# jason2714/de-i2i-gan

Measured on AMD Instinct MI355X. Metric: paired 256x256 images/sec (G+D train step), higher is better.
Workload: dtype bf16

## Files before the change

### de-i2i-gan_amd/csrc/conv_api.hip

```cpp
#include <hip/hip_runtime.h>

#include "../../include/dei2i_hip.h"
#include "launch.h"

namespace dei2i {

static ConvShape to_shape(const dei2i_conv* c) {
  ConvShape s;
  s.N = c->N; s.H = c->H; s.W = c->W; s.Cin = c->Cin; s.Cout = c->Cout;
  s.kh = c->kh; s.kw = c->kw; s.stride = c->stride; s.pad = c->pad; s.pad_mode = c->pad_mode; s.up = c->up;
  return s;
}

static bool valid_conv(const dei2i_conv* c) {
  if (!c) return false;
  const int vec = c->dtype == DT_BF16 ? 8 : 4;
  if (c->dtype != DT_BF16 && c->dtype != DT_F32) return false;
  if (c->N <= 0 || c->H <= 0 || c->W <= 0 || c->Cin <= 0 || c->Cout <= 0) return false;
  if (c->CinS < c->Cin || c->CoutS < c->Cout || c->CinS % vec || c->CoutS % vec) return false;
  if (c->kh <= 0 || c->kw <= 0 || c->stride <= 0 || c->pad < 0 || c->up < 0 || c->up > 1) return false;
  if (c->kh < c->stride || c->kw < c->stride) return false;
  if (c->pad_mode == PAD_REFLECT && (c->pad >= (c->H << c->up) || c->pad >= (c->W << c->up))) return false;
  if (((c->H << c->up) + 2 * c->pad) < c->kh || ((c->W << c->up) + 2 * c->pad) < c->kw) return false;
  return true;
// ... 335 lines not shown
    hipError_t e = gather_gemm(c->dtype, interior, dy, wd_packed, c->Cin, nullptr, dx, ws, ws_bytes, c->CinS, ACT_NONE, st);
    if (e != hipSuccess) return (int)e;
    GatherDesc ring[4];
    reflect_ring_descs(ring_frame, c->H, c->W, p, c->kh, c->kw, ring);
    const long long woffs[4] = {0, 0, 0, 0};
    e = gather_gemm_multi(c->dtype, ring, woffs, 4, dy, wd_packed, c->Cin, nullptr, ext_scratch, ws, ws_bytes, c->CinS, ACT_NONE, st,
                          true);
    if (e != hipSuccess) return (int)e;
    return fold_border(c, ext_scratch, dx, p, st);
  }
  if (reflect && g_opt.dgrad_s2_ring && c->stride == 2 && c->kh == 4 && c->kw == 4 && p == 1 && !c->up && c->H % 2 == 0 && c->W % 2 == 0 &&
      c->H >= 8 && c->W >= 8 && (size_t)c->N * c->H * c->W * c->CinS >= ((size_t)48 << 20)) {
    ConvShape sh = to_shape(c);
    GatherDesc rows[4], cols[4], in4[4];
    long long wrows4[4], wcols4[4], woffs[4];
    s2_ring_descs(sh, c->CoutS, rows, wrows4, cols, wcols4);
    sh.pad_mode = PAD_ZERO;
    for_each_dgrad_class(c->Cin, c->CoutS, c->kh, c->kw, 2, [&](const DgradClass& k) {
      in4[2 * k.ay + k.ax] = make_dgrad_desc(sh, c->CoutS, k.ay, k.ax);
      woffs[2 * k.ay + k.ax] = k.off;
    });
    hipError_t e = gather_gemm_multi(c->dtype, in4, woffs, 4, dy, wd_packed, c->Cin, nullptr, dx, ws, ws_bytes, c->CinS, ACT_NONE, st);
    if (e != hipSuccess) return (int)e;
    e = gather_gemm_multi(c->dtype, rows, wrows4, 4, dy, wd_packed, c->Cin, nullptr, ext_scratch, ws, ws_bytes, c->CinS, ACT_NONE, st, true);
    if (e != hipSuccess) return (int)e;
    e = gather_gemm_multi(c->dtype, cols, wcols4, 4, dy, wd_packed, c->Cin, nullptr, ext_scratch, ws, ws_bytes, c->CinS, ACT_NONE, st, true);
    if (e != hipSuccess) return (int)e;
    return fold_border(c, ext_scratch, dx, 1, st);
  }
  const int rc = dei2i_conv2d_dgrad(c, dy, wd_packed, ext_scratch, ws, ws_bytes, s);
  if (rc != 0) return rc;
  return dei2i_fold_pad(c->dtype, c->N, c->H, c->W, c->CinS, c->pad, c->pad_mode, c->up, ext_scratch, nullptr, dx, s);
}

static GatherDesc interior_dgrad_desc(const dei2i_conv* c) {
  ConvShape sh = to_shape(c);
  sh.pad_mode = PAD_ZERO;
  return make_dgrad_desc(sh, c->CoutS, 0, 0);
}

static bool dgrad_norm_shape_ok(const dei2i_conv* c) {
  if (!g_opt.halo16 || !g_opt.halo16_fold) return false;
  if (!valid_conv(c) || c->dtype != DT_BF16 || c->up) return false;
  if (c->kh != 3 || c->kw != 3 || c->stride != 1 || c->pad != 1 || c->pad_mode != PAD_REFLECT) return false;
  return halo16_shape_ok(interior_dgrad_desc(c), c->CinS, true, true, false);
}

int dei2i_conv2d_dgrad_norm_supported(const dei2i_conv* c) { return dgrad_norm_shape_ok(c) ? 1 : 0; }

int dei2i_conv2d_dgrad_norm_chunks(const dei2i_conv* c) { return (c->H / 16) * (c->W / 32); }

int dei2i_conv2d_dgrad_input_norm(const dei2i_conv* c, const void* dy, const void* wd_packed, void* dx, const dei2i_epi_norm* en,
                                  dei2i_stream s) {
  if (!dy || !wd_packed || !dx || !en || !dgrad_norm_shape_ok(c)) return DEI2I_ERR_BAD_ARG;
  if (!en->x || !en->mean || !en->rstd || !en->partial || en->up < 0 || en->up > 1) return DEI2I_ERR_BAD_ARG;
  const int kind = en->kind;
  if (kind == 1 ? !en->gb : (kind != 2 || !en->a || !en->b || en->up)) return DEI2I_ERR_BAD_ARG;
  if (en->group_images < 0 || (en->group_images > 0 && c->N % en->group_images != 0)) return DEI2I_ERR_BAD_ARG;
  const GatherDesc interior = interior_dgrad_desc(c);
  EpiNorm e;
  e.x = (const uint16_t*)en->x; e.mean = en->mean; e.rstd = en->rstd; e.gb = (const uint16_t*)en->gb; e.a = en->a; e.b = en->b;
  e.partial = en->partial; e.kind = en->kind; e.up = en->up; e.act = en->act;
  e.group_images = kind == 2 ? en->group_images : 0;
  hipError_t ef = halo16_conv(interior, dy, wd_packed, c->Cin, nullptr, dx, c->CinS, ACT_NONE, (hipStream_t)s, nullptr, nullptr, true, &e);
  return ef == hipErrorNotSupported ? DEI2I_ERR_BAD_ARG : (int)ef;
}

int dei2i_conv2d_wgrad_oihw(const dei2i_conv* c, const void* x, const void* dy, float* scratch, size_t scratch_elems,
                            float* dw_oihw, int accumulate, dei2i_stream s) {
  if (!valid_conv(c) || !x || !dy || !scratch || !dw_oihw) return DEI2I_ERR_BAD_ARG;
  hipStream_t st = (hipStream_t)s;
  GatherDesc g = make_fwd_desc(to_shape(c), c->CinS);
  const size_t packed = (size_t)wgrad_slab_elems(c->Cout, g.K);
  if (scratch_elems < packed) return DEI2I_ERR_WORKSPACE;
  const bool bf16 = c->dtype == DT_BF16;
  int nsplit = 0;
  hipError_t e = hipErrorNotSupported;
  if (bf16 && g_opt.wgrad_thin)
    e = wgrad_thin(g, x, dy, c->Cout, c->CoutS, scratch, scratch_elems, &nsplit, st);
  if (e == hipErrorNotSupported && bf16 && g_opt.wgrad_halo)
    e = wgrad_halo(g, x, dy, c->Cout, c->CoutS, scratch, scratch_elems, &nsplit, g_opt.wgrad_halo == 2, st);
  if (e == hipErrorNotSupported && bf16 && g_opt.wgrad_v2)
    e = wgrad_v2(g, x, dy, c->Cout, c->CoutS, scratch, scratch_elems, &nsplit, st);
  if (e == hipErrorNotSupported) e = wgrad_gemm(c->dtype, g, x, dy, c->Cout, c->CoutS, scratch, scratch_elems, &nsplit, st);
  if (e != hipSuccess) return (int)e;
  return (int)wgrad_reduce_unpack(scratch, nsplit, (long long)packed, dw_oihw, c->Cout, c->Cin, c->CinS, c->kh * c->kw, accumulate, st);
}

static bool to_pro(const dei2i_conv* c, const dei2i_pro* p, ConvPro& out) {
  if (p == nullptr) return false;
  out.A = p->A; out.B = p->B; out.n_stride = p->n_stride; out.slope = p->slope;
  out.ring = (const uint16_t*)p->ring;
  out.ring_pix = p->ring != nullptr ? ring_pixels(c->H << c->up, c->W << c->up) : 0;
  return true;
}

static bool halo_fwd_shape_ok(const dei2i_conv* c, int want_pro) {
  if (!valid_conv(c) || c->dtype != DT_BF16) return false;
  if (c->kh == 4 && c->kw == 4 && c->stride == 2 && c->pad == 1 && !want_pro)
    return halo16_s2_shape_ok(make_fwd_desc(to_shape(c), c->CinS), c->CoutS);
  if (c->kh != 3 || c->kw != 3 || c->stride != 1 || c->pad != 1) return false;
  return halo_conv_shape_ok(make_fwd_desc(to_shape(c), c->CinS), c->CoutS, want_pro != 0, want_pro != 0);
}

int dei2i_conv2d_fused_supported(const dei2i_conv* c, int want_pro) { return halo_fwd_shape_ok(c, want_pro) ? 1 : 0; }

int dei2i_conv2d_stats_chunks(const dei2i_conv* c) {
  int Ho, Wo;
  dei2i_conv2d_out_shape(c, &Ho, &Wo);
  return (Ho / 8) * (Wo / 32);
}

int dei2i_conv2d_fwd_fused(const dei2i_conv* c, const void* x, const void* w_packed, const float* bias, int act, void* y,
                           const dei2i_pro* pro, float* stats, dei2i_stream s) {
  if (!x || !w_packed || !y || !halo_fwd_shape_ok(c, pro != nullptr)) return DEI2I_ERR_BAD_ARG;
  if (pro != nullptr && (!pro->A || !pro->B)) return DEI2I_ERR_BAD_ARG;
  GatherDesc g = make_fwd_desc(to_shape(c), c->CinS);
  ConvPro cp;
  const bool has = to_pro(c, pro, cp);
  if (!has) {
    hipError_t e = halo16_conv(g, x, w_packed, c->Cout, bias, y, c->CoutS, act, (hipStream_t)s, stats);
    if (e != hipErrorNotSupported) return (int)e;
  }
  return (int)halo_conv(g, x, w_packed, c->Cout, bias, y, c->CoutS, act, (hipStream_t)s, nullptr, has ? &cp : nullptr, stats);
}

int dei2i_conv2d_ring_supported(const dei2i_conv* c) {
  if (!halo_fwd_shape_ok(c, 0) || !c->up) return 0;
  return halo16_shape_ok(make_fwd_desc(to_shape(c), c->CinS), c->CoutS, false, false, true) ? 1 : 0;
}

int dei2i_conv2d_fwd_ring(const dei2i_conv* c, const void* z_src, const void* ring, const void* w_packed, const float* bias, int act,
                          void* y, float* stats, dei2i_stream s) {
  if (!z_src || !ring || !w_packed || !y || !dei2i_conv2d_ring_supported(c)) return DEI2I_ERR_BAD_ARG;
  GatherDesc g = make_fwd_desc(to_shape(c), c->CinS);
  return (int)halo16_conv(g, z_src, w_packed, c->Cout, bias, y, c->CoutS, act, (hipStream_t)s, stats, ring);
}

int dei2i_conv2d_wgrad_pro_supported(const dei2i_conv* c) {
  if (!valid_conv(c) || c->dtype != DT_BF16) return 0;
  if (c->kh != 3 || c->kw != 3 || c->stride != 1 || c->pad != 1) return 0;
  return wgrad_halo_shape_ok(make_fwd_desc(to_shape(c), c->CinS), c->Cout, true) != 0 ? 1 : 0;
}

int dei2i_conv2d_wgrad_oihw_pro(const dei2i_conv* c, const void* x, const void* dy, float* scratch, size_t scratch_elems,
                                float* dw_oihw, int accumulate, const dei2i_pro* pro, dei2i_stream s) {
  if (!x || !dy || !scratch || !dw_oihw || !pro || !dei2i_conv2d_wgrad_pro_supported(c)) return DEI2I_ERR_BAD_ARG;
  if ((pro->A == nullptr) != (pro->B == nullptr) || (pro->A == nullptr && pro->ring == nullptr)) return DEI2I_ERR_BAD_ARG;
  hipStream_t st = (hipStream_t)s;
  GatherDesc g = make_fwd_desc(to_shape(c), c->CinS);
  const size_t packed = (size_t)wgrad_slab_elems(c->Cout, g.K);
  if (scratch_elems < packed) return DEI2I_ERR_WORKSPACE;
  ConvPro cp;
  to_pro(c, pro, cp);
  int nsplit = 0;
  hipError_t e = wgrad_halo(g, x, dy, c->Cout, c->CoutS, scratch, scratch_elems, &nsplit, true, st, &cp);
  if (e != hipSuccess) return (int)e;
  return (int)wgrad_reduce_unpack(scratch, nsplit, (long long)packed, dw_oihw, c->Cout, c->Cin, c->CinS, c->kh * c->kw, accumulate, st);
}

int dei2i_fold_pad(int dtype, int N, int H, int W, int C, int pad, int pad_mode, int up, const void* dx_ext,
                   const void* addend, void* dx, dei2i_stream s) {
  const int vec = dtype == DT_BF16 ? 8 : 4;
  if (N <= 0 || H <= 0 || W <= 0 || C <= 0 || C % vec || pad < 0 || pad > 3 || up < 0 || up > 1 || !dx_ext || !dx)
    return DEI2I_ERR_BAD_ARG;
  const size_t total = (size_t)N * H * W * (C / vec);
  const unsigned grid = grid_for(total, 256, 256u * 16u);
  const int reflect = (pad_mode == PAD_REFLECT && pad > 0) ? 1 : 0;
// ... 10 lines not shown
```

### de-i2i-gan_amd/csrc/conv_gemm.hip

```cpp
#include <hip/hip_runtime.h>
#include <stdint.h>
#include <stdio.h>
#include <algorithm>

#include "common.h"
#include "geom.h"
#include "launch.h"

namespace dei2i {

template <typename T> struct Mma;
template <> struct Mma<bf16_t> {
  static DEI2I_D void run(const u32x4& a, const u32x4& b, f32x16& c) {
    c = __builtin_amdgcn_mfma_f32_32x32x16_bf16(__builtin_bit_cast(bf16x8, a), __builtin_bit_cast(bf16x8, b), c, 0, 0, 0);
  }
};
template <> struct Mma<float> {
  static DEI2I_D void run(const u32x4& a, const u32x4& b, f32x16& c) {
    c = __builtin_amdgcn_mfma_f32_32x32x2f32(__uint_as_float(a.x), __uint_as_float(b.x), c, 0, 0, 0);
    c = __builtin_amdgcn_mfma_f32_32x32x2f32(__uint_as_float(a.y), __uint_as_float(b.y), c, 0, 0, 0);
    c = __builtin_amdgcn_mfma_f32_32x32x2f32(__uint_as_float(a.z), __uint_as_float(b.z), c, 0, 0, 0);
    c = __builtin_amdgcn_mfma_f32_32x32x2f32(__uint_as_float(a.w), __uint_as_float(b.w), c, 0, 0, 0);
  }
};
// ... 189 lines not shown
  constexpr int NV = BN / 4;
#pragma unroll 1
  for (int v = tid; v < BM * NV; v += 256) {
    const int row = v / NV, n = n0 + (v - row * NV) * 4;
    const int m = m0 + row;
    if (m >= g.M || n >= ldc) continue;
    const f32x4 q = *reinterpret_cast<const f32x4*>(stg + row * SROW + (n - n0));
    if (ws != nullptr) {
      const size_t wrow = (size_t)(pack.m_base[blockIdx.y] + m);
      *reinterpret_cast<f32x4*>(ws + ((size_t)blockIdx.z * slab_rows + wrow) * ldc + n) = q;
      continue;
    }
    size_t opix;
    if (g.out_identity) {
      opix = (size_t)m;
    } else {
      int ni, oy, ox;
      decode_m(g, m, ni, oy, ox);
      opix = (size_t)out_pixel(g, ni, oy, ox);
    }
    float o[4] = {q.x, q.y, q.z, q.w};
#pragma unroll
    for (int e = 0; e < 4; ++e) {
      if (n + e < wrows) {
        if (bias != nullptr) o[e] += bias[n + e];
        o[e] = apply_act(o[e], act);
      } else {
        o[e] = 0.f;
      }
    }
    T* dst = out + opix * ldc + n;
    if constexpr (sizeof(T) == 2) {
      u32x2 pk;
      pk.x = (uint32_t)f32_to_bf16(o[0]) | ((uint32_t)f32_to_bf16(o[1]) << 16);
      pk.y = (uint32_t)f32_to_bf16(o[2]) | ((uint32_t)f32_to_bf16(o[3]) << 16);
      *reinterpret_cast<u32x2*>(dst) = pk;
    } else {
      f32x4 pk = {o[0], o[1], o[2], o[3]};
      *reinterpret_cast<f32x4*>(dst) = pk;
    }
  }
}

template <typename T>
__global__ void splitk_finalize_kernel(const DescPack pack, const float* __restrict__ ws, const int zs, const size_t slab_elems,
                                       const float* __restrict__ bias, T* __restrict__ out, int ldc, int co, int act) {
  size_t q = (size_t)blockIdx.x * blockDim.x + threadIdx.x;
  const size_t stride = (size_t)gridDim.x * blockDim.x;
  const size_t total4 = slab_elems >> 2;
  for (; q < total4; q += stride) {
    const size_t i = q << 2;
    const int c = (int)(i % (size_t)ldc);
    const int r = (int)(i / (size_t)ldc);
    int k = 0;
    while (k + 1 < pack.n && r >= pack.m_base[k + 1]) ++k;
    const GatherDesc& g = pack.d[k];
    int n, oy, ox;
    decode_m(g, r - pack.m_base[k], n, oy, ox);
    const size_t opix = (size_t)out_pixel(g, n, oy, ox);
    f32x4 v0 = {0.f, 0.f, 0.f, 0.f}, v1 = v0;
    if (c < co) {
      int z = 0;
      for (; z + 1 < zs; z += 2) {
        v0 += *reinterpret_cast<const f32x4*>(ws + (size_t)z * slab_elems + i);
        v1 += *reinterpret_cast<const f32x4*>(ws + (size_t)(z + 1) * slab_elems + i);
      }
      if (z < zs) v0 += *reinterpret_cast<const f32x4*>(ws + (size_t)z * slab_elems + i);
    }
    const f32x4 v = v0 + v1;
    const float vv[4] = {v.x, v.y, v.z, v.w};
#pragma unroll
    for (int e = 0; e < 4; ++e) {
      float o = 0.f;
      if (c + e < co) {
        o = vv[e];
        if (bias != nullptr) o += bias[c + e];
        o = apply_act(o, act);
      }
      Elem<T>::store(out + opix * ldc + c + e, o);
    }
  }
}

template <int ROWB> DEI2I_D int tr_swz(int row) {
  if constexpr (ROWB % 256 == 0) return (row & 3) << 6;
  else return ((row >> 1) & 1) << 6;
}

template <typename T, int BM, int BN>
__global__ __launch_bounds__(256) void wgrad_kernel(const GatherDesc g, const T* __restrict__ src,
                                                    const T* __restrict__ dy, const int co_rows, const int ldy,
                                                    float* __restrict__ dw_base, const int tiles_k,
                                                    const int chunks_per_split, const long long slab_elems) {
  constexpr int VEC = Elem<T>::VEC;
  constexpr bool IS_BF16 = sizeof(T) == 2;
  float* __restrict__ dw = dw_base + (size_t)blockIdx.z * (size_t)slab_elems;
  constexpr int BR = 128 / (int)sizeof(T);
  constexpr int VPR_A = BM / VEC, VPR_B = BN / VEC;
  constexpr int RPP_A = 256 / VPR_A, RPP_B = 256 / VPR_B;
  constexpr int NA = BR / RPP_A, NB = BR / RPP_B;
  constexpr int ROWB_A = BM * (int)sizeof(T), ROWB_B = BN * (int)sizeof(T);
  constexpr int WTM = BM / 2, WTN = BN / 2;
  constexpr int TM = WTM / 32, TN = WTN / 32;
  static_assert(NA >= 1 && NB >= 1, "tile too wide for 256 threads");
  static_assert(TM >= 1 && TN >= 1, "wave tile must hold at least one 32x32 block");

  extern __shared__ __attribute__((aligned(16))) unsigned char smem[];
  constexpr int A_BYTES = BR * ROWB_A, B_BYTES = BR * ROWB_B;
  constexpr int TILE_BYTES = A_BYTES + B_BYTES;

  const int tid = threadIdx.x, lane = tid & 63, wave = tid >> 6;
  const int wm = wave >> 1, wn = wave & 1;
  const int nwg = gridDim.x;
  const int bid = xcd_remap(blockIdx.x, nwg);
  const int tile_k = bid % tiles_k, tile_c = bid / tiles_k;
  const int c0 = tile_c * BM, k0 = tile_k * BN;

  const int nchunks = (g.M + BR - 1) / BR;
  const int cbeg = blockIdx.z * chunks_per_split;
  const int cend = min(nchunks, cbeg + chunks_per_split);
  if (cbeg >= cend) return;

  const int va = tid % VPR_A, ra0 = tid / VPR_A;
  const int a_c = c0 + va * VEC;
  const bool a_cok = a_c < ldy;
  const int vb = tid % VPR_B, rb0 = tid / VPR_B;
  const int b_k = k0 + vb * VEC;
  const bool b_kok = b_k < g.K;
  int b_tap, b_ci;
  decode_k(g, b_kok ? b_k : 0, b_tap, b_ci);
  const int b_ty = (int)fd_div((uint32_t)b_tap, g.fd_tw);
  const int b_dy = b_ty * g.ys, b_dx = (b_tap - b_ty * g.tw) * g.xs;

  u32x4 areg[NA], breg[NB];
  auto load_chunk = [&](int chunk) {
    const int mb = chunk * BR;
#pragma unroll
    for (int i = 0; i < NA; ++i) {
      const int m = mb + ra0 + RPP_A * i;
      areg[i] = (a_cok && m < g.M) ? ld16(dy + (size_t)m * ldy + a_c) : zero16();
    }
#pragma unroll
    for (int i = 0; i < NB; ++i) {
      const int m = mb + rb0 + RPP_B * i;
      u32x4 v = zero16();
      if (b_kok && m < g.M) {
        int n, oy, ox;
        decode_m(g, m, n, oy, ox);
        const int y = bound_coord(oy * g.sh + g.by0 + b_dy, g.Hl, g.pad_mode);
        const int x = bound_coord(ox * g.sw + g.bx0 + b_dx, g.Wl, g.pad_mode);
        if ((y | x) >= 0) {
          const int pix = (n * g.Hs + (y >> g.up)) * g.Ws + (x >> g.up);
          v = ld16(src + (size_t)pix * g.Cs + b_ci);
        }
      }
      breg[i] = v;
    }
  };
  auto store_chunk = [&](int buf) {
    unsigned char* ab = smem + buf * TILE_BYTES;
    unsigned char* bb = ab + A_BYTES;
#pragma unroll
    for (int i = 0; i < NA; ++i) {
      const int row = ra0 + RPP_A * i;
      int off = va * 16;
      if (IS_BF16) off ^= tr_swz<ROWB_A>(row);
      *reinterpret_cast<u32x4*>(ab + row * ROWB_A + off) = areg[i];
    }
#pragma unroll
    for (int i = 0; i < NB; ++i) {
      const int row = rb0 + RPP_B * i;
      int off = vb * 16;
      if (IS_BF16) off ^= tr_swz<ROWB_B>(row);
      *reinterpret_cast<u32x4*>(bb + row * ROWB_B + off) = breg[i];
    }
  };

  f32x16 acc[TM][TN];
#pragma unroll
  for (int i = 0; i < TM; ++i)
#pragma unroll
    for (int j = 0; j < TN; ++j)
#pragma unroll
      for (int e = 0; e < 16; ++e) acc[i][j][e] = 0.f;

  const int lr = lane & 31, lh = lane >> 5;
  const int tr_q = (lane & 15) >> 2, tr_p = lane & 3, tr_cohalf = (lane >> 4) & 1;

  auto compute_chunk = [&](int buf) {
    const unsigned char* ab = smem + buf * TILE_BYTES;
    const unsigned char* bb = ab + A_BYTES;
    if constexpr (IS_BF16) {
      u32x4 af[BR / 16][TM], bf[BR / 16][TN];
      auto load_frags = [&](int kk, u32x4 (&a)[TM], u32x4 (&b)[TN]) {
        const int row_lo = kk * 16 + 8 * lh + tr_q;
#pragma unroll
        for (int i = 0; i < TM; ++i) {
          const int colb = (wm * WTM + i * 32 + 16 * tr_cohalf + 4 * tr_p) * 2;
          const int o0 = row_lo * ROWB_A + (colb ^ tr_swz<ROWB_A>(row_lo));
          const int o1 = (row_lo + 4) * ROWB_A + (colb ^ tr_swz<ROWB_A>(row_lo + 4));
          s16x4 lo = __builtin_amdgcn_ds_read_tr16_b64_v4i16((__attribute__((address_space(3))) s16x4*)(ab + o0));
          s16x4 hi = __builtin_amdgcn_ds_read_tr16_b64_v4i16((__attribute__((address_space(3))) s16x4*)(ab + o1));
          u32x2 l2 = __builtin_bit_cast(u32x2, lo), h2 = __builtin_bit_cast(u32x2, hi);
          a[i].x = l2.x; a[i].y = l2.y; a[i].z = h2.x; a[i].w = h2.y;
        }
#pragma unroll
        for (int j = 0; j < TN; ++j) {
          const int colb = (wn * WTN + j * 32 + 16 * tr_cohalf + 4 * tr_p) * 2;
          const int o0 = row_lo * ROWB_B + (colb ^ tr_swz<ROWB_B>(row_lo));
          const int o1 = (row_lo + 4) * ROWB_B + (colb ^ tr_swz<ROWB_B>(row_lo + 4));
          s16x4 lo = __builtin_amdgcn_ds_read_tr16_b64_v4i16((__attribute__((address_space(3))) s16x4*)(bb + o0));
          s16x4 hi = __builtin_amdgcn_ds_read_tr16_b64_v4i16((__attribute__((address_space(3))) s16x4*)(bb + o1));
          u32x2 l2 = __builtin_bit_cast(u32x2, lo), h2 = __builtin_bit_cast(u32x2, hi);
          b[j].x = l2.x; b[j].y = l2.y; b[j].z = h2.x; b[j].w = h2.y;
        }
      };
#pragma unroll
      for (int kk = 0; kk < BR / 16; ++kk) load_frags(kk, af[kk], bf[kk]);
#pragma unroll
      for (int kk = 0; kk < BR / 16; ++kk) {
#pragma unroll
        for (int i = 0; i < TM; ++i)
#pragma unroll
          for (int j = 0; j < TN; ++j)
            acc[i][j] = __builtin_amdgcn_mfma_f32_32x32x16_bf16(__builtin_bit_cast(bf16x8, af[kk][i]),
                                                                 __builtin_bit_cast(bf16x8, bf[kk][j]), acc[i][j], 0, 0, 0);
      }
    } else {
#pragma unroll 4
      for (int kk = 0; kk < BR / 2; ++kk) {
        float af[TM], bf[TN];
        const int row = kk * 2 + lh;
#pragma unroll
        for (int i = 0; i < TM; ++i)
          af[i] = *reinterpret_cast<const float*>(ab + row * ROWB_A + (wm * WTM + i * 32 + lr) * 4);
#pragma unroll
        for (int j = 0; j < TN; ++j)
          bf[j] = *reinterpret_cast<const float*>(bb + row * ROWB_B + (wn * WTN + j * 32 + lr) * 4);
#pragma unroll
        for (int i = 0; i < TM; ++i)
#pragma unroll
          for (int j = 0; j < TN; ++j)
            acc[i][j] = __builtin_amdgcn_mfma_f32_32x32x2f32(af[i], bf[j], acc[i][j], 0, 0, 0);
      }
    }
  };

  {
    int buf = 1;
#pragma unroll 1
    for (int c = cbeg; c <= cend; ++c) {
      const bool more = c < cend;
      if (more) load_chunk(c);
      if (c > cbeg) compute_chunk(buf);
      if (more) store_chunk(buf ^ 1);
      __syncthreads();
      buf ^= 1;
    }
  }

#pragma unroll
  for (int i = 0; i < TM; ++i)
#pragma unroll
    for (int q = 0; q < 4; ++q) {
      const int co = c0 + wm * WTM + i * 32 + 8 * q + 4 * lh;
      if (co >= co_rows) continue;
#pragma unroll
      for (int j = 0; j < TN; ++j) {
        const int k = k0 + wn * WTN + j * 32 + lr;
        if (k < g.K) {
          float* p = dw + (size_t)co * g.K + k;
#pragma unroll
          for (int r = 0; r < 4; ++r) p[(size_t)r * g.K] = acc[i][j][q * 4 + r];
        }
      }
    }
}

template <typename T, int BM, int BN, int WM, int WN>
static hipError_t launch_gg(const DescPack& pack, const void* src, const void* wgt, int wrows, const float* bias,
                            void* out, float* ws, int ldc, int act, int splits, int slab_rows, int* zs_out, hipStream_t st) {
  constexpr int BKE = 128 / (int)sizeof(T);
  int tiles_m = 0, Kmax = 0;
  double flops = 0.0;
  for (int i = 0; i < pack.n; ++i) {
    const GatherDesc& g = pack.d[i];
    tiles_m = std::max(tiles_m, (g.M + BM - 1) / BM);
    Kmax = std::max(Kmax, g.K);
    flops += conv_flops(g, wrows);
  }
  if (pack.skip_dead_taps) flops = 0.0;
  const int tiles_n = (ldc + BN - 1) / BN;
  const int nk = (Kmax + BKE - 1) / BKE;
  const int kps = (nk + splits - 1) / splits;
  const int zs = (nk + kps - 1) / kps;
  dim3 grid(tiles_m * tiles_n, pack.n, zs);
  const size_t lds = std::max<size_t>(2 * (BM + BN) * 128, (size_t)BM * (BN + 4) * sizeof(float));
  *zs_out = zs;
  return launch_counted(K_GATHER_V1, PROF_GATHER_GEMM, flops, gather_gemm_kernel<T, BM, BN, WM, WN>, grid, dim3(256), lds, st, pack,
                        (const T*)src, (const T*)wgt, wrows, bias, (T*)out, zs > 1 ? ws : (float*)nullptr, ldc, act, tiles_n, kps,
                        slab_rows);
}

template <typename T>
static hipError_t gather_gemm_t(const DescPack& pack, const void* src, const void* wgt, int wrows, const float* bias,
                                void* out, float* ws, size_t ws_bytes, int ldc, int act, hipStream_t st) {
  constexpr int BKE = 128 / (int)sizeof(T);
  int BN = ldc > 64 ? 128 : (ldc > 32 ? 64 : 32);
  const int BM = 128;
  int tiles = 0, nk = 0;
  bool any = false;
  for (int i = 0; i < pack.n; ++i) {
    const GatherDesc& g = pack.d[i];
    if (g.M <= 0) continue;
    any = true;
    tiles += ((g.M + BM - 1) / BM) * ((ldc + BN - 1) / BN);
    nk = std::max(nk, (g.K + BKE - 1) / BKE);
  }
  if (!any) return hipSuccess;
  const GatherDesc& g0 = pack.d[0];
  const int slab_rows = pack.m_base[pack.n - 1] + pack.d[pack.n - 1].M;
  const size_t slab_elems = (size_t)slab_rows * ldc;
  int splits = 1;
  if (tiles < num_cu() && nk >= 4 && ws != nullptr && ws_bytes >= 2 * slab_elems * sizeof(float)) {
    splits = (2 * num_cu() + tiles - 1) / tiles;
    if (splits > nk / 2) splits = nk / 2;
    const size_t fit = ws_bytes / (slab_elems * sizeof(float));
    if ((size_t)splits > fit) splits = (int)fit;
    if (splits < 1) splits = 1;
  }
  if (splits > 1 && !pack.ws_compact && (long long)slab_rows < (long long)g0.N * g0.OH * g0.OW) {
    hipError_t e0 = hipMemsetAsync(out, 0, (size_t)g0.N * g0.OH * g0.OW * ldc * sizeof(T), st);
    if (e0 != hipSuccess) return e0;
  }
  hipError_t e;
  int zs = 1;
  if (BN == 128) e = launch_gg<T, 128, 128, 2, 2>(pack, src, wgt, wrows, bias, out, ws, ldc, act, splits, slab_rows, &zs, st);
  else if (BN == 64) e = launch_gg<T, 128, 64, 2, 2>(pack, src, wgt, wrows, bias, out, ws, ldc, act, splits, slab_rows, &zs, st);
  else e = launch_gg<T, 128, 32, 4, 1>(pack, src, wgt, wrows, bias, out, ws, ldc, act, splits, slab_rows, &zs, st);
  if (e != hipSuccess) return e;
  if (zs > 1) {
    const int threads = 256;
    size_t blocks = ((slab_elems >> 2) + threads - 1) / threads;
    if (blocks > 4096) blocks = 4096;
    count_launch(K_SPLITK_FINALIZE);
    hipLaunchKernelGGL(splitk_finalize_kernel<T>, dim3((unsigned)blocks), dim3(threads), 0, st, pack, (const float*)ws,
                       zs, slab_elems, bias, (T*)out, ldc, wrows, act);
    e = hipGetLastError();
  }
  return e;
}

hipError_t gather_gemm_multi(int dtype, const GatherDesc* descs, const long long* woffs, int n, const void* src,
                             const void* wgt, int wrows, const float* bias, void* out, float* ws, size_t ws_bytes, int ldc,
                             int act, hipStream_t st, bool compact_ws) {
  if (n < 1 || n > 4) return hipErrorInvalidValue;
  DescPack pack;
  pack.n = 0;
  pack.ws_compact = compact_ws ? 1 : 0;
  pack.skip_dead_taps = compact_ws ? 1 : 0;
  for (int i = 0; i < n; ++i) {
    if (descs[i].M <= 0) continue;
    pack.d[pack.n] = descs[i];
    pack.woff[pack.n] = woffs[i];
    pack.fd_taps[pack.n] = make_fastdiv((uint32_t)(descs[i].th * descs[i].tw));
    pack.m_base[pack.n] = pack.n == 0 ? 0 : pack.m_base[pack.n - 1] + pack.d[pack.n - 1].M;
    pack.n++;
  }
  if (pack.n == 0) return hipSuccess;
  for (int i = pack.n; i < 4; ++i) { pack.d[i] = pack.d[0]; pack.woff[i] = 0; pack.fd_taps[i] = pack.fd_taps[0]; pack.m_base[i] = 0; }
  if (dtype == DT_BF16) {
    if (g_opt.thin_conv && pack.n == 1) {
      hipError_t e = thin_cin_conv(pack.d[0], src, (const bf16_t*)wgt + pack.woff[0], wrows, bias, out, ldc, act, st);
      if (e != hipErrorNotSupported) return e;
      e = thin_cout_conv(pack.d[0], src, (const bf16_t*)wgt + pack.woff[0], wrows, bias, out, ldc, act, st);
      if (e != hipErrorNotSupported) return e;
    }
    if (g_opt.halo_conv && pack.n == 1) {
      hipError_t e = halo16_conv(pack.d[0], src, (const bf16_t*)wgt + pack.woff[0], wrows, bias, out, ldc, act, st);
      if (e != hipErrorNotSupported) return e;
      e = halo_conv(pack.d[0], src, (const bf16_t*)wgt + pack.woff[0],
                               wrows, bias, out, ldc, act, st);
      if (e != hipErrorNotSupported) return e;
    }
    if (g_opt.gather_gemm_v2) {
      hipError_t e = gather_gemm_v2(pack, src, wgt, wrows, bias, out, ws, ws_bytes, ldc, act, st);
      if (e != hipErrorNotSupported) return e;
    }
    return gather_gemm_t<bf16_t>(pack, src, wgt, wrows, bias, out, ws, ws_bytes, ldc, act, st);
  }
  return gather_gemm_t<float>(pack, src, wgt, wrows, bias, out, ws, ws_bytes, ldc, act, st);
}

hipError_t gather_gemm(int dtype, const GatherDesc& g, const void* src, const void* wgt, int wrows, const float* bias,
                       void* out, float* ws, size_t ws_bytes, int ldc, int act, hipStream_t st) {
  const long long zero = 0;
  return gather_gemm_multi(dtype, &g, &zero, 1, src, wgt, wrows, bias, out, ws, ws_bytes, ldc, act, st);
}

template <typename T, int BM, int BN>
static hipError_t launch_wg(const GatherDesc& g, const void* src, const void* dy, int co_rows, int ldy, float* dw,
                            size_t capacity_elems, int* nsplit_out, hipStream_t st) {
  constexpr int BR = 128 / (int)sizeof(T);
  const int tiles_c = (co_rows + BM - 1) / BM;
  const int tiles_k = (g.K + BN - 1) / BN;
  const int nchunks = (g.M + BR - 1) / BR;
  const int tiles = tiles_c * tiles_k;
  int splits = (2 * num_cu() + tiles - 1) / tiles;
  if (splits > nchunks / 2) splits = nchunks / 2;
  const long long slab_elems = wgrad_slab_elems(co_rows, g.K);
  if ((size_t)slab_elems * (size_t)splits > capacity_elems) splits = (int)(capacity_elems / (size_t)slab_elems);
  if (splits < 1) splits = 1;
  const int cps = (nchunks + splits - 1) / splits;
  const int zs = (nchunks + cps - 1) / cps;
  const size_t lds = 2 * (size_t)BR * (BM + BN) * sizeof(T);
  *nsplit_out = zs;
  return launch_counted(K_WGRAD_V1, PROF_WGRAD, conv_flops(g, co_rows), wgrad_kernel<T, BM, BN>, dim3(tiles, 1, zs), dim3(256), lds, st,
                        g, (const T*)src, (const T*)dy, co_rows, ldy, dw, tiles_k, cps, slab_elems);
}

hipError_t wgrad_gemm(int dtype, const GatherDesc& g, const void* src, const void* dy, int co_rows, int ldy, float* dw,
                      size_t capacity_elems, int* nsplit_out, hipStream_t st) {
  if (g.M <= 0) {
    *nsplit_out = 0;
    return hipSuccess;
  }
  if (dtype == DT_BF16) {
    if (co_rows > 64) return launch_wg<bf16_t, 128, 128>(g, src, dy, co_rows, ldy, dw, capacity_elems, nsplit_out, st);
    return launch_wg<bf16_t, 64, 128>(g, src, dy, co_rows, ldy, dw, capacity_elems, nsplit_out, st);
  }
  if (co_rows > 64) return launch_wg<float, 128, 128>(g, src, dy, co_rows, ldy, dw, capacity_elems, nsplit_out, st);
  return launch_wg<float, 64, 128>(g, src, dy, co_rows, ldy, dw, capacity_elems, nsplit_out, st);
}

}
```

### de-i2i-gan_amd/csrc/launch.h

```cpp
#pragma once
#include <hip/hip_runtime.h>
#include <stddef.h>
#include <stdint.h>

#include "common.h"
#include "geom.h"

namespace dei2i {

enum ProfFamily : int { PROF_GATHER_GEMM = 0, PROF_WGRAD = 1, PROF_HALO_CONV = 2, PROF_HALO_FOLD = 3, PROF_FAMILIES = 4 };
enum KernelId : int { K_GATHER_V1 = 0, K_GATHER_V2, K_HALO_CONV, K_HALO_CONV_FP8, K_THIN_CIN, K_THIN_COUT, K_WGRAD_V1, K_WGRAD_V2,
                      K_WGRAD_HALO, K_WGRAD_THIN, K_HALO16_CONV, K_SPLITK_FINALIZE, K_HALO16_S2, K_COUNT };
void count_launch(int kid);
void prof_begin(int family, double flops, hipStream_t st);
void prof_end(int family, hipStream_t st);

struct Options {
  int gather_gemm_v2 = 1;
  int wgrad_v2 = 1;
  int halo_conv = 1;
  int thin_conv = 1;
  int halo16 = 1;
  int halo16_fold = 1;
  int halo16_s2 = 1;
  int wgrad_halo = 1;
  int wgrad_thin = 1;
  int dgrad_s2_ring = 1;
  int num_cu = 256;
};
extern Options g_opt;
inline int num_cu() { return g_opt.num_cu; }

inline double conv_flops(const GatherDesc& g, int rows) {
  return 2.0 * (double)g.M * (double)(g.th * g.tw) * (double)g.Clog * (double)rows;
}

hipError_t ensure_dyn_lds(const void* kernel, size_t bytes);

template <typename... KArgs, typename... Args>
static inline hipError_t launch_counted(int kid, int family, double flops, void (*kern)(KArgs...), dim3 grid, dim3 block,
                                        size_t lds, hipStream_t st, Args&&... args) {
  hipError_t e = ensure_dyn_lds(reinterpret_cast<const void*>(kern), lds);
  if (e != hipSuccess) return e;
  count_launch(kid);
  prof_begin(family, flops, st);
  hipLaunchKernelGGL(kern, grid, block, lds, st, args...);
  prof_end(family, st);
  return hipGetLastError();
}

struct DescPack {
  GatherDesc d[4];
  long long woff[4];
  FastDiv fd_taps[4];
  int n;
  int ws_compact;
  int skip_dead_taps;
  int m_base[4];
};

hipError_t gather_gemm_v2(const DescPack& pack, const void* src, const void* wgt, int wrows, const float* bias, void* out,
                          float* ws, size_t ws_bytes, int ldc, int act, hipStream_t st);
hipError_t thin_cout_conv(const GatherDesc& g, const void* src, const void* wgt, int wrows, const float* bias, void* out, int ldc,
                          int act, hipStream_t st);
hipError_t thin_cin_conv(const GatherDesc& g, const void* src, const void* wgt, int wrows, const float* bias, void* out, int ldc,
                         int act, hipStream_t st);
bool halo_conv_shape_ok(const GatherDesc& g, int ldc, bool pro, bool pro_ring);
hipError_t halo_conv(const GatherDesc& g, const void* src, const void* wgt, int wrows, const float* bias, void* out, int ldc,
                     int act, hipStream_t st, const float* dequant = nullptr, const ConvPro* pro = nullptr,
                     float* stats = nullptr);

hipError_t halo16_conv(const GatherDesc& g, const void* src, const void* wgt, int wrows, const float* bias, void* out, int ldc,
                       int act, hipStream_t st, float* stats = nullptr, const void* ring = nullptr, bool fold = false,
                       const EpiNorm* en = nullptr);
bool halo16_shape_ok(const GatherDesc& g, int ldc, bool fold, bool epin, bool ring);
bool halo16_s2_shape_ok(const GatherDesc& g, int ldc);
hipError_t gather_gemm(int dtype, const GatherDesc& g, const void* src, const void* wgt, int wrows, const float* bias,
                       void* out, float* ws, size_t ws_bytes, int ldc, int act, hipStream_t st);
hipError_t gather_gemm_multi(int dtype, const GatherDesc* descs, const long long* woffs, int n, const void* src,
                             const void* wgt, int wrows, const float* bias, void* out, float* ws, size_t ws_bytes, int ldc,
                             int act, hipStream_t st, bool compact_ws = false);
static inline long long wgrad_slab_elems(int co_rows, int K) { return (long long)((co_rows + 7) & ~7) * K; }
hipError_t wgrad_gemm(int dtype, const GatherDesc& g, const void* src, const void* dy, int co_rows, int ldy, float* dw,
                      size_t capacity_elems, int* nsplit_out, hipStream_t st);

hipError_t wgrad_v2(const GatherDesc& g, const void* src, const void* dy, int co_rows, int ldy, float* slabs,
                    size_t slab_capacity_elems, int* nsplit_out, hipStream_t st);
int wgrad_halo_shape_ok(const GatherDesc& g, int co_rows, bool pro_ring);
hipError_t wgrad_halo(const GatherDesc& g, const void* src, const void* dy, int co_rows, int ldy, float* slabs,
                      size_t slab_capacity_elems, int* nsplit_out, bool force, hipStream_t st,
                      const ConvPro* pro = nullptr);
hipError_t wgrad_thin(const GatherDesc& g, const void* src, const void* dy, int co_rows, int ldy, float* slabs,
                      size_t slab_capacity_elems, int* nsplit_out, hipStream_t st);
hipError_t wgrad_reduce_unpack(float* slabs, int nsplit, long long slab_elems, float* dw, int Cout, int Cin, int CinS,
                               int taps, int accumulate, hipStream_t st);

template <typename F>
static inline void by_dtype(int dtype, F&& f) {
  if (dtype == DT_BF16) f(bf16_t{});
  else f(float{});
}

inline unsigned grid_for(size_t work_items, int threads, unsigned cap = 256u * 8u) {
  size_t b = (work_items + threads - 1) / threads;
  if (b < 1) b = 1;
  if (b > cap) b = cap;
  return (unsigned)b;
}

}
```

### de-i2i-gan_amd/csrc/runtime.hip

```cpp
#include <hip/hip_runtime.h>
#include <mutex>
#include <string.h>
#include <vector>

#include "../../include/dei2i_hip.h"
#include "launch.h"

namespace dei2i {

Options g_opt;

struct LdsLimit { const void* kernel; size_t bytes; };
static LdsLimit g_lds_limits[64];
static int g_lds_kernels = 0;
static std::mutex g_lds_mutex;

hipError_t ensure_dyn_lds(const void* kernel, size_t bytes) {
  std::lock_guard<std::mutex> lock(g_lds_mutex);
  int i = 0;
  while (i < g_lds_kernels && g_lds_limits[i].kernel != kernel) ++i;
  if (i < g_lds_kernels && bytes <= g_lds_limits[i].bytes) return hipSuccess;
  hipError_t e = hipFuncSetAttribute(kernel, hipFuncAttributeMaxDynamicSharedMemorySize, (int)bytes);
  if (e != hipSuccess) return e;
  if (i == g_lds_kernels && g_lds_kernels < 64) g_lds_limits[g_lds_kernels++] = LdsLimit{kernel, 0};
  if (i < g_lds_kernels) g_lds_limits[i].bytes = bytes;
  return hipSuccess;
}

struct ProfState {
  bool on = false;
  bool events = true;
  int every = 1;
  bool armed = false;
  double flops_timed = 0.0;
  size_t counted = 0;
  std::vector<hipEvent_t> starts, stops;
  size_t used = 0;
  double flops = 0.0;
};
static ProfState g_prof[PROF_FAMILIES];

static long long g_launches[K_COUNT];
void count_launch(int kid) { g_launches[kid]++; }
static const char* const g_kernel_names[] = {"gather_v1", "gather_v2", "halo_conv", "halo_conv_fp8", "thin_cin", "thin_cout",
                                             "wgrad_v1", "wgrad_v2", "wgrad_halo", "wgrad_thin", "halo16_conv", "splitk_finalize", "halo16_s2"};
static_assert(sizeof(g_kernel_names) / sizeof(g_kernel_names[0]) == K_COUNT, "one name per KernelId, in its order");

static const struct { const char* name; int Options::*member; } g_option_table[] = {
    {"gather_gemm_v2", &Options::gather_gemm_v2}, {"wgrad_v2", &Options::wgrad_v2},     {"halo_conv", &Options::halo_conv},
    {"thin_conv", &Options::thin_conv},           {"halo16", &Options::halo16},         {"halo16_fold", &Options::halo16_fold},
    {"halo16_s2", &Options::halo16_s2},           {"wgrad_halo", &Options::wgrad_halo}, {"wgrad_thin", &Options::wgrad_thin},
    {"dgrad_s2_ring", &Options::dgrad_s2_ring}};

void prof_begin(int family, double flops, hipStream_t st) {
  ProfState& p = g_prof[family];
  if (!p.on) return;
  p.counted++;
  p.flops += flops;
  p.armed = p.events && (p.counted - 1) % (size_t)p.every == 0;
  if (!p.armed) return;
  p.flops_timed += flops;
  if (p.used == p.starts.size()) {
    hipEvent_t a, b;
    hipEventCreate(&a);
    hipEventCreate(&b);
    p.starts.push_back(a);
    p.stops.push_back(b);
  }
  hipEventRecord(p.starts[p.used], st);
}

void prof_end(int family, hipStream_t st) {
  ProfState& p = g_prof[family];
  if (!p.on || !p.armed) return;
  hipEventRecord(p.stops[p.used], st);
  p.used++;
}

}

using namespace dei2i;

extern "C" {

int dei2i_version(void) { return 100; }

int dei2i_init(int device) {
  hipDeviceProp_t prop;
  hipError_t e = hipGetDeviceProperties(&prop, device);
  if (e != hipSuccess) return (int)e;
  g_opt.num_cu = prop.multiProcessorCount > 0 ? prop.multiProcessorCount : 256;
  return 0;
}

const char* dei2i_error_string(int code) {
  if (code == DEI2I_ERR_BAD_ARG) return "dei2i: bad argument";
  if (code == DEI2I_ERR_WORKSPACE) return "dei2i: workspace too small";
  if (code >= 0) return hipGetErrorString((hipError_t)code);
  return "dei2i: unknown error";
}

int dei2i_set_option(const char* name, int value) {
  if (name == nullptr) return DEI2I_ERR_BAD_ARG;
  for (const auto& o : g_option_table)
    if (strcmp(name, o.name) == 0) { g_opt.*o.member = value; return 0; }
  return DEI2I_ERR_BAD_ARG;
}

int dei2i_launch_counts(int64_t* out, int n) {
  for (int i = 0; i < n && i < K_COUNT; ++i) out[i] = (int64_t)g_launches[i];
  return K_COUNT;
}
void dei2i_launch_counts_reset(void) { for (int i = 0; i < K_COUNT; ++i) g_launches[i] = 0; }
const char* dei2i_kernel_name(int kid) { return kid >= 0 && kid < K_COUNT ? g_kernel_names[kid] : nullptr; }

int dei2i_prof_enable(int family, int on) {
  if (family < 0 || family >= PROF_FAMILIES) return DEI2I_ERR_BAD_ARG;
  ProfState& p = g_prof[family];
  p.on = on != 0;
  p.events = on != 2;
  p.every = on >= 3 ? on : 1;
  p.used = 0;
  p.counted = 0;
  p.flops = 0.0;
  p.flops_timed = 0.0;
  return 0;
}

int dei2i_prof_collect_timed(int family, int64_t* timed_launches, double* timed_flops) {
  if (family < 0 || family >= PROF_FAMILIES) return DEI2I_ERR_BAD_ARG;
  if (timed_launches) *timed_launches = (int64_t)g_prof[family].used;
  if (timed_flops) *timed_flops = g_prof[family].flops_timed;
  return 0;
}

// ... 24 lines not shown
```

Measured before the change: 476.1.

## Write wgrad tiles directly to OIHW and widen split-K finalize reduction

When the wgrad GEMM needs only one slab and a tile covers exactly one channel vector across all taps, the kernel stages its fp32 accumulator tile in LDS, permutes it to OIHW order and writes or accumulates straight into dw. This removes the separate reduce/unpack kernel and the slab round trip through memory. Separately, split-K finalize with many slices and few output vectors now gives each vector several lanes and combines their partial sums with a shuffle reduction. Both paths are on by default through new options and are limited to specific shapes, which adds template variants and extra LDS reuse.

Result: no change. 478.5 (median of 6 runs) (+0.5%).

```diff
diff --git a/de-i2i-gan_amd/csrc/conv_api.hip b/de-i2i-gan_amd/csrc/conv_api.hip
--- a/de-i2i-gan_amd/csrc/conv_api.hip
+++ b/de-i2i-gan_amd/csrc/conv_api.hip
@@ -441,8 +441,9 @@
     e = wgrad_halo(g, x, dy, c->Cout, c->CoutS, scratch, scratch_elems, &nsplit, g_opt.wgrad_halo == 2, st);
   if (e == hipErrorNotSupported && bf16 && g_opt.wgrad_v2)
     e = wgrad_v2(g, x, dy, c->Cout, c->CoutS, scratch, scratch_elems, &nsplit, st);
-  if (e == hipErrorNotSupported) e = wgrad_gemm(c->dtype, g, x, dy, c->Cout, c->CoutS, scratch, scratch_elems, &nsplit, st);
-  if (e != hipSuccess) return (int)e;
+  WgradDirect direct{dw_oihw, c->Cin, accumulate, false};
+  if (e == hipErrorNotSupported) e = wgrad_gemm(c->dtype, g, x, dy, c->Cout, c->CoutS, scratch, scratch_elems, &nsplit, st, &direct);
+  if (e != hipSuccess || direct.done) return (int)e;
   return (int)wgrad_reduce_unpack(scratch, nsplit, (long long)packed, dw_oihw, c->Cout, c->Cin, c->CinS, c->kh * c->kw, accumulate, st);
 }
 
diff --git a/de-i2i-gan_amd/csrc/conv_gemm.hip b/de-i2i-gan_amd/csrc/conv_gemm.hip
--- a/de-i2i-gan_amd/csrc/conv_gemm.hip
+++ b/de-i2i-gan_amd/csrc/conv_gemm.hip
@@ -295,16 +295,59 @@
   }
 }
 
+template <typename T>
+__global__ __launch_bounds__(256) void splitk_finalize_wide_kernel(const DescPack pack, const float* __restrict__ ws, const int zs,
+                                                                   const size_t slab_elems, const float* __restrict__ bias,
+                                                                   T* __restrict__ out, int ldc, int co, int act, const int G) {
+  const size_t t = (size_t)blockIdx.x * blockDim.x + threadIdx.x;
+  const size_t q = t / (size_t)G;
+  const int j = (int)(t - q * (size_t)G);
+  const bool live = q < (slab_elems >> 2);
+  const size_t i = q << 2;
+  const int c = live ? (int)(i % (size_t)ldc) : 0;
+  f32x4 v = {0.f, 0.f, 0.f, 0.f};
+  if (live && c < co) {
+#pragma unroll 4
+    for (int z = j; z < zs; z += G) v += *reinterpret_cast<const f32x4*>(ws + (size_t)z * slab_elems + i);
+  }
+  for (int o = G >> 1; o > 0; o >>= 1) {
+    v.x += __shfl_xor(v.x, o);
+    v.y += __shfl_xor(v.y, o);
+    v.z += __shfl_xor(v.z, o);
+    v.w += __shfl_xor(v.w, o);
+  }
+  if (!live || j != 0) return;
+  const int r = (int)(i / (size_t)ldc);
+  int k = 0;
+  while (k + 1 < pack.n && r >= pack.m_base[k + 1]) ++k;
+  const GatherDesc& g = pack.d[k];
+  int n, oy, ox;
+  decode_m(g, r - pack.m_base[k], n, oy, ox);
+  const size_t opix = (size_t)out_pixel(g, n, oy, ox);
+  const float vv[4] = {v.x, v.y, v.z, v.w};
+#pragma unroll
+  for (int e = 0; e < 4; ++e) {
+    float o = 0.f;
+    if (c + e < co) {
+      o = vv[e];
+      if (bias != nullptr) o += bias[c + e];
+      o = apply_act(o, act);
+    }
+    Elem<T>::store(out + opix * ldc + c + e, o);
+  }
+}
+
 template <int ROWB> DEI2I_D int tr_swz(int row) {
   if constexpr (ROWB % 256 == 0) return (row & 3) << 6;
   else return ((row >> 1) & 1) << 6;
 }
 
-template <typename T, int BM, int BN>
+template <typename T, int BM, int BN, bool DIRECT>
 __global__ __launch_bounds__(256) void wgrad_kernel(const GatherDesc g, const T* __restrict__ src,
                                                     const T* __restrict__ dy, const int co_rows, const int ldy,
                                                     float* __restrict__ dw_base, const int tiles_k,
-                                                    const int chunks_per_split, const long long slab_elems) {
+                                                    const int chunks_per_split, const long long slab_elems,
+                                                    float* __restrict__ dw_oihw, const int Cin, const int accumulate) {
   constexpr int VEC = Elem<T>::VEC;
   constexpr bool IS_BF16 = sizeof(T) == 2;
   float* __restrict__ dw = dw_base + (size_t)blockIdx.z * (size_t)slab_elems;
@@ -339,9 +382,14 @@
   const bool a_cok = a_c < ldy;
   const int vb = tid % VPR_B, rb0 = tid / VPR_B;
   const int b_k = k0 + vb * VEC;
-  const bool b_kok = b_k < g.K;
+  const bool b_kok = DIRECT ? tile_k * VEC < g.Cs : b_k < g.K;
   int b_tap, b_ci;
-  decode_k(g, b_kok ? b_k : 0, b_tap, b_ci);
+  if constexpr (DIRECT) {
+    b_tap = vb;
+    b_ci = tile_k * VEC;
+  } else {
+    decode_k(g, b_kok ? b_k : 0, b_tap, b_ci);
+  }
   const int b_ty = (int)fd_div((uint32_t)b_tap, g.fd_tw);
   const int b_dy = b_ty * g.ys, b_dx = (b_tap - b_ty * g.tw) * g.xs;
 
@@ -472,6 +520,35 @@
     }
   }
 
+  if constexpr (DIRECT) {
+    constexpr int TAPS = BN / VEC;
+    static_assert(BM * BN * (int)sizeof(float) <= 2 * TILE_BYTES, "the fp32 tile fits the operand buffers");
+    float* __restrict__ stg = reinterpret_cast<float*>(smem);
+#pragma unroll
+    for (int i = 0; i < TM; ++i)
+#pragma unroll
+      for (int e = 0; e < 16; ++e) {
+        const int row = wm * WTM + i * 32 + (e & 3) + 8 * (e >> 2) + 4 * lh;
+#pragma unroll
+        for (int j = 0; j < TN; ++j) {
+          const int c = wn * WTN + j * 32 + lr;
+          stg[row * BN + (c % VEC) * TAPS + c / VEC] = acc[i][j][e];
+        }
+      }
+    __syncthreads();
+    const int ci0 = tile_k * VEC;
+#pragma unroll 1
+    for (int v = tid; v < BM * (BN / 4); v += 256) {
+      const int row = v / (BN / 4), p = (v - row * (BN / 4)) * 4;
+      const int co = c0 + row, ci = ci0 + p / TAPS;
+      if (co >= co_rows || ci >= Cin) continue;
+      float* o = dw_oihw + ((size_t)co * Cin + ci) * TAPS + p % TAPS;
+      f32x4 q = *reinterpret_cast<const f32x4*>(stg + row * BN + p);
+      if (accumulate) q += *reinterpret_cast<const f32x4*>(o);
+      *reinterpret_cast<f32x4*>(o) = q;
+    }
+    return;
+  }
 #pragma unroll
   for (int i = 0; i < TM; ++i)
 #pragma unroll
@@ -557,8 +634,16 @@
     size_t blocks = ((slab_elems >> 2) + threads - 1) / threads;
     if (blocks > 4096) blocks = 4096;
     count_launch(K_SPLITK_FINALIZE);
-    hipLaunchKernelGGL(splitk_finalize_kernel<T>, dim3((unsigned)blocks), dim3(threads), 0, st, pack, (const float*)ws,
-                       zs, slab_elems, bias, (T*)out, ldc, wrows, act);
+    int G = 1;
+    while (g_opt.finalize_wide && G < 64 && zs >= 8 * G && (slab_elems >> 2) * (size_t)(2 * G) <= (size_t)65536) G *= 2;
+    if (G >= 4) {
+      const size_t wide_blocks = ((slab_elems >> 2) * (size_t)G + threads - 1) / threads;
+      hipLaunchKernelGGL(splitk_finalize_wide_kernel<T>, dim3((unsigned)wide_blocks), dim3(threads), 0, st, pack, (const float*)ws,
+                         zs, slab_elems, bias, (T*)out, ldc, wrows, act, G);
+    } else {
+      hipLaunchKernelGGL(splitk_finalize_kernel<T>, dim3((unsigned)blocks), dim3(threads), 0, st, pack, (const float*)ws,
+                         zs, slab_elems, bias, (T*)out, ldc, wrows, act);
+    }
     e = hipGetLastError();
   }
   return e;
@@ -613,7 +698,7 @@
 
 template <typename T, int BM, int BN>
 static hipError_t launch_wg(const GatherDesc& g, const void* src, const void* dy, int co_rows, int ldy, float* dw,
-                            size_t capacity_elems, int* nsplit_out, hipStream_t st) {
+                            size_t capacity_elems, int* nsplit_out, WgradDirect* direct, hipStream_t st) {
   constexpr int BR = 128 / (int)sizeof(T);
   const int tiles_c = (co_rows + BM - 1) / BM;
   const int tiles_k = (g.K + BN - 1) / BN;
@@ -628,22 +713,31 @@
   const int zs = (nchunks + cps - 1) / cps;
   const size_t lds = 2 * (size_t)BR * (BM + BN) * sizeof(T);
   *nsplit_out = zs;
-  return launch_counted(K_WGRAD_V1, PROF_WGRAD, conv_flops(g, co_rows), wgrad_kernel<T, BM, BN>, dim3(tiles, 1, zs), dim3(256), lds, st,
-                        g, (const T*)src, (const T*)dy, co_rows, ldy, dw, tiles_k, cps, slab_elems);
+  if constexpr (sizeof(T) == 2) {
+    if (g_opt.wgrad_direct && direct != nullptr && zs == 1 && g.th * g.tw * Elem<T>::VEC == BN &&
+        reinterpret_cast<uintptr_t>(direct->dw) % 16 == 0) {
+      direct->done = true;
+      return launch_counted(K_WGRAD_V1, PROF_WGRAD, conv_flops(g, co_rows), wgrad_kernel<T, BM, BN, true>, dim3(tiles, 1, 1), dim3(256),
+                            lds, st, g, (const T*)src, (const T*)dy, co_rows, ldy, dw, tiles_k, cps, slab_elems, direct->dw, direct->Cin,
+                            direct->accumulate);
+    }
+  }
+  return launch_counted(K_WGRAD_V1, PROF_WGRAD, conv_flops(g, co_rows), wgrad_kernel<T, BM, BN, false>, dim3(tiles, 1, zs), dim3(256), lds,
+                        st, g, (const T*)src, (const T*)dy, co_rows, ldy, dw, tiles_k, cps, slab_elems, (float*)nullptr, 0, 0);
 }
 
 hipError_t wgrad_gemm(int dtype, const GatherDesc& g, const void* src, const void* dy, int co_rows, int ldy, float* dw,
-                      size_t capacity_elems, int* nsplit_out, hipStream_t st) {
+                      size_t capacity_elems, int* nsplit_out, hipStream_t st, WgradDirect* direct) {
   if (g.M <= 0) {
     *nsplit_out = 0;
     return hipSuccess;
   }
   if (dtype == DT_BF16) {
-    if (co_rows > 64) return launch_wg<bf16_t, 128, 128>(g, src, dy, co_rows, ldy, dw, capacity_elems, nsplit_out, st);
-    return launch_wg<bf16_t, 64, 128>(g, src, dy, co_rows, ldy, dw, capacity_elems, nsplit_out, st);
-  }
-  if (co_rows > 64) return launch_wg<float, 128, 128>(g, src, dy, co_rows, ldy, dw, capacity_elems, nsplit_out, st);
-  return launch_wg<float, 64, 128>(g, src, dy, co_rows, ldy, dw, capacity_elems, nsplit_out, st);
-}
-
-}
+    if (co_rows > 64) return launch_wg<bf16_t, 128, 128>(g, src, dy, co_rows, ldy, dw, capacity_elems, nsplit_out, direct, st);
+    return launch_wg<bf16_t, 64, 128>(g, src, dy, co_rows, ldy, dw, capacity_elems, nsplit_out, direct, st);
+  }
+  if (co_rows > 64) return launch_wg<float, 128, 128>(g, src, dy, co_rows, ldy, dw, capacity_elems, nsplit_out, direct, st);
+  return launch_wg<float, 64, 128>(g, src, dy, co_rows, ldy, dw, capacity_elems, nsplit_out, direct, st);
+}
+
+}
diff --git a/de-i2i-gan_amd/csrc/launch.h b/de-i2i-gan_amd/csrc/launch.h
--- a/de-i2i-gan_amd/csrc/launch.h
+++ b/de-i2i-gan_amd/csrc/launch.h
@@ -26,6 +26,8 @@
   int wgrad_halo = 1;
   int wgrad_thin = 1;
   int dgrad_s2_ring = 1;
+  int finalize_wide = 1;
+  int wgrad_direct = 1;
   int num_cu = 256;
 };
 extern Options g_opt;
@@ -81,8 +83,14 @@
                              const void* wgt, int wrows, const float* bias, void* out, float* ws, size_t ws_bytes, int ldc,
                              int act, hipStream_t st, bool compact_ws = false);
 static inline long long wgrad_slab_elems(int co_rows, int K) { return (long long)((co_rows + 7) & ~7) * K; }
+struct WgradDirect {
+  float* dw;
+  int Cin;
+  int accumulate;
+  bool done;
+};
 hipError_t wgrad_gemm(int dtype, const GatherDesc& g, const void* src, const void* dy, int co_rows, int ldy, float* dw,
-                      size_t capacity_elems, int* nsplit_out, hipStream_t st);
+                      size_t capacity_elems, int* nsplit_out, hipStream_t st, WgradDirect* direct = nullptr);
 
 hipError_t wgrad_v2(const GatherDesc& g, const void* src, const void* dy, int co_rows, int ldy, float* slabs,
                     size_t slab_capacity_elems, int* nsplit_out, hipStream_t st);
diff --git a/de-i2i-gan_amd/csrc/runtime.hip b/de-i2i-gan_amd/csrc/runtime.hip
--- a/de-i2i-gan_amd/csrc/runtime.hip
+++ b/de-i2i-gan_amd/csrc/runtime.hip
@@ -50,7 +50,8 @@
     {"gather_gemm_v2", &Options::gather_gemm_v2}, {"wgrad_v2", &Options::wgrad_v2},     {"halo_conv", &Options::halo_conv},
     {"thin_conv", &Options::thin_conv},           {"halo16", &Options::halo16},         {"halo16_fold", &Options::halo16_fold},
     {"halo16_s2", &Options::halo16_s2},           {"wgrad_halo", &Options::wgrad_halo}, {"wgrad_thin", &Options::wgrad_thin},
-    {"dgrad_s2_ring", &Options::dgrad_s2_ring}};
+    {"dgrad_s2_ring", &Options::dgrad_s2_ring},   {"wgrad_direct", &Options::wgrad_direct},
+    {"finalize_wide", &Options::finalize_wide}};
 
 void prof_begin(int family, double flops, hipStream_t st) {
   ProfState& p = g_prof[family];
diff --git a/profiles/small_m_table.py b/profiles/small_m_table.py
--- /dev/null
+++ b/profiles/small_m_table.py
@@ -0,0 +1,69 @@
+#!/usr/bin/env python3
+import collections
+import csv
+import sys
+
+ROWS = [
+    ("D5 fwd N=64 | D4 fwd N=32", "gather_v1 128x128, 4 k-slices", "gather_gemm_kernel<unsigned short, 128, 128", (128, 1, 4), 68.7, 83.9),
+    ("D5 fwd N=32", "gather_v1 128x128, 8 k-slices", "gather_gemm_kernel<unsigned short, 128, 128", (64, 1, 8), 34.4, 73.4),
+    ("D5 | D4(N=32) fwd finalize", "splitk_finalize", "splitk_finalize_kernel<unsigned short>", (2048, 1, 1), 0.0, 37.7),
+    ("finalize at 1024 workgroups (D5 fwd N=32 is one of six)", "splitk_finalize", "splitk_finalize_kernel<unsigned short>", (1024, 1, 1), 0.0, 35.7),
+    ("D4 fwd N=64", "gather_v2 256x128", "gather_gemm_v2_kernel<256, 128, 4, 2, 3>", (128, 1, 1), 68.7, 41.9),
+    ("D5 dgrad N=64", "gather_v2 256x128, 4 classes", "gather_gemm_v2_kernel<256, 128, 4, 2, 3>", (56, 4, 1), 107.4, 88.6),
+    ("D5 dgrad N=32", "gather_v2 192x128, 4 classes", "gather_gemm_v2_kernel<192, 128, 2, 4, 3>", (40, 4, 1), 53.7, 75.8),
+    ("D4 dgrad N=64", "gather_v2 256x256, 4 classes", "gather_gemm_v2_kernel<256, 256, 2, 4, 2>", (42, 4, 1), 87.0, 46.7),
+    ("D4 dgrad N=32", "gather_v2 192x128, 4 classes", "gather_gemm_v2_kernel<192, 128, 2, 4, 3>", (56, 4, 1), 43.5, 31.7),
+    ("D5 wgrad N=64", "wgrad_v1 128x128, one slab", "wgrad_kernel<unsigned short, 128, 128", (2048, 1, 1), 68.7, 146.8),
+    ("D5 wgrad un-pack", "wgrad_reduce_unpack (1 slab)", "wgrad_reduce_unpack_kernel", (2048, 16, 1), 0.0, 268.4),
+    ("D4 wgrad N=64", "wgrad_v2 256x128, one slab", "wgrad_v2_kernel<256>", (256, 1, 1), 68.7, 50.3),
+    ("D4 wgrad un-pack", "wgrad_reduce_unpack (1 slab)", "wgrad_reduce_unpack_kernel", (1024, 8, 1), 0.0, 67.1),
+    ("src_clf fwd N=64", "gather_v1 128x32, 58 k-slices", "gather_gemm_kernel<unsigned short, 128, 32", (8, 1, 58), 0.04, 4.2),
+    ("src_clf fwd N=64 finalize", "splitk_finalize, 58 slices of 2048 vectors", "splitk_finalize_kernel<unsigned short>", (8, 1, 1), 0.0, 1.9),
+    ("cls_clf fwd N=64 | N=32", "gather_v1 128x32, 256 k-slices", "gather_gemm_kernel<unsigned short, 128, 32", (1, 1, 256), 0.05, 4.7),
+    ("cls_clf fwd finalize", "splitk_finalize, 256 slices of <= 128 vectors", "splitk_finalize_kernel<unsigned short>", (1, 1, 1), 0.0, 0.5),
+    ("src_clf wgrad N=64", "wgrad_v1 64x128, 4 slabs", "wgrad_kernel<unsigned short, 64, 128", (144, 1, 4), 0.04, 4.3),
+    ("cls_clf wgrad N=64", "wgrad_v1 64x128, one slab", "wgrad_kernel<unsigned short, 64, 128", (256, 1, 1), 0.05, 4.7),
+    ("cls_clf wgrad un-pack", "wgrad_reduce_unpack (1 slab)", "wgrad_reduce_unpack_kernel", (6, 32, 1), 0.0, 1.6),
+]
+
+
+def main(trace, out):
+    launches = collections.defaultdict(list)
+    steps = 7
+    for r in csv.DictReader(open(trace)):
+        name = r["Kernel_Name"]
+        if "dei2i::" not in name:
+            continue
+        grid = (int(r["Grid_Size_X"]) // int(r["Workgroup_Size_X"]), int(r["Grid_Size_Y"]) // int(r["Workgroup_Size_Y"]),
+                int(r["Grid_Size_Z"]) // int(r["Workgroup_Size_Z"]))
+        launches[(name.split("(")[0], grid)].append((int(r["End_Timestamp"]) - int(r["Start_Timestamp"])) / 1000.0)
+    with open(out, "w", newline="") as f:
+        w = csv.writer(f)
+        w.writerow(["shape", "kernel", "instance", "grid", "launches_per_step", "min_us", "median_us", "max_us", "us_per_step",
+                    "flop_floor_us", "byte_floor_us"])
+        for shape, what, sub, grid, gflop, mb in ROWS:
+            hits = [(k, v) for k, v in launches.items() if sub in k[0] and k[1] == grid]
+            if "finalize" in sub and not hits:
+                continue
+            for (kname, kgrid), ts in hits:
+                ts = sorted(ts)
+                w.writerow([shape, what, kname.replace("void dei2i::", ""), "x".join(map(str, kgrid)), round(len(ts) / steps, 2),
+                            round(ts[0], 1), round(ts[len(ts) // 2], 1), round(ts[-1], 1), round(sum(ts) / steps, 1),
+                            round(gflop * 1e9 / 2.5e15 * 1e6, 1), round(mb * 1e6 / 4.5e12 * 1e6, 1)])
+        for (kname, kgrid), ts in sorted(launches.items()):
+            if "splitk_finalize_wide" in kname:
+                ts = sorted(ts)
+                w.writerow(["heads fwd finalize", "splitk_finalize, several lanes per vector", kname.replace("void dei2i::", ""),
+                            "x".join(map(str, kgrid)), round(len(ts) / steps, 2), round(ts[0], 1), round(ts[len(ts) // 2], 1),
+                            round(ts[-1], 1), round(sum(ts) / steps, 1), 0.0, ""])
+        fams = ["gather_gemm_kernel", "splitk_finalize", "wgrad_kernel", "wgrad_reduce_unpack"]
+        total = 0.0
+        for fam in fams:
+            t = sum(sum(v) for k, v in launches.items() if fam in k[0]) / steps
+            total += t
+            w.writerow(["family sum", fam, "", "", "", "", "", "", round(t, 1), "", ""])
+        w.writerow(["family sum", "the four families", "", "", "", "", "", "", round(total, 1), "", ""])
+
+
+if __name__ == "__main__":
+    main(sys.argv[1], sys.argv[2])
```
